# Kitware/SMQTK-Indexing

Measured on AMD Instinct MI355X. Metric: queries/sec, exact brute-force l2 kNN k=100 over 10000000x128 float32 (recall@100 = 1.0 by construction); scan HBM GB/s vs 8 TB/s peak, higher is better.
Workload: dtype f32 results (distances bit-identical to numpy float32); filter arithmetic int8 MFMA (i32 accumulation, measured per-row error bound), exact re-rank f32

## Files before the change

### smqtk_indexing_amd/csrc/sq_dense_i8.hpp

```cpp
#pragma once
#include "sq_dense_scan.hpp"

namespace sq {

typedef int i32x4 __attribute__((ext_vector_type(4)));
typedef int i32x16 __attribute__((ext_vector_type(16)));

template <int KS>
struct I8Geom {
    static constexpr int ROW_BYTES = KS * 32;
    static constexpr int UNIT_ROWS = KS == 4 ? 64 : 32;
    static constexpr int TILES = UNIT_ROWS / 32;
    static constexpr int UNIT_BYTES = UNIT_ROWS * ROW_BYTES;
    static constexpr int SLOT_BYTES = UNIT_BYTES + 256;
    static constexpr int WAVES = KS <= 8 ? 8 : 4;
    static constexpr int NSTAGE = 2;
    static constexpr int PIECES = UNIT_BYTES / 1024;
    static constexpr int SAMPLES_PER_UNIT = 2 * TILES;
};
static constexpr int I8_MAX_ROW_BYTES = 512;
__host__ __device__ constexpr int i8_row_bytes(int d) { return d <= 128 ? 128 : (d <= 256 ? 256 : 512); }
__host__ __device__ constexpr int i8_unit_rows(int row_bytes) { return row_bytes == 128 ? 64 : 32; }

__device__ __forceinline__ float i8_element(float v, const float* __restrict__ center, int k, bool cosine, double inv_norm) {
// ... 84 lines not shown
            }
        }
        if (__ballot(bad) != 0ull) continue;
#pragma unroll
        for (int c = 0; c < I8_NCLIP; ++c) {
            for (int o = 32; o > 0; o >>= 1) r2[c] += __shfl_xor(r2[c], o);
#pragma unroll
            for (int m = 0; m < I8_NCUT; ++m) cnt[c][m] += r2[c] > ca.cut[c][m] ? 1u : 0u;
        }
    }
    if (lane == 0) {
#pragma unroll
        for (int c = 0; c < I8_NCLIP; ++c)
#pragma unroll
            for (int m = 0; m < I8_NCUT; ++m)
                if (cnt[c][m]) atomicAdd(&counts[c * I8_NCUT + m], cnt[c][m]);
    }
}

template <int EPL>
static __global__ __launch_bounds__(256) void dense8_build_kernel(const float* __restrict__ db, long long n, long long ld, int d,
                                                                   long long n_pad, const float* __restrict__ center,
                                                                   const double* __restrict__ nx64, float inv_dx, float dx,
                                                                   signed char* __restrict__ out8, float* __restrict__ nrow,
                                                                   float* __restrict__ r2row, long long row_base, int row_bytes) {
    const int lane = threadIdx.x & 63;
    const long long row = row_base + (long long)blockIdx.x * 4 + (threadIdx.x >> 6);
    if (row >= n_pad) return;
    double e2 = 0.0, r2 = 0.0;
    bool finite = true;
    const double inv_norm = (row < n && nx64) ? 1.0 / sqrt(nx64[row]) : 1.0;
    for (int k0 = 0; k0 < row_bytes; k0 += 64 * EPL) {
        unsigned char q[EPL];
#pragma unroll
        for (int j = 0; j < EPL; ++j) q[j] = 0;
        if (row < n) {
#pragma unroll
            for (int j = 0; j < EPL; ++j) {
                const int k = k0 + EPL * lane + j;
                if (k < d) {
                    const float v = db[row * ld + k];
                    const float xc = i8_element(v, center, k, nx64 != nullptr, inv_norm);
                    if (!(xc == xc) || !(fabsf(xc) < 3.0e38f)) finite = false;
                    float t = rintf(xc * inv_dx);
                    t = fminf(fmaxf(t, -127.f), 127.f);
                    if (!(t == t)) t = 0.f;
                    q[j] = (unsigned char)(signed char)(int)t;
                    const double res = (double)xc - (double)t * (double)dx;
                    e2 += (double)xc * (double)xc;
                    r2 += res * res;
                }
            }
        }
        if (k0 + EPL * lane >= row_bytes) continue;
        unsigned char* dst = reinterpret_cast<unsigned char*>(out8) + row * row_bytes + k0 + EPL * lane;
        if constexpr (EPL == 2) {
            *reinterpret_cast<unsigned short*>(dst) = (unsigned short)(q[0] | (q[1] << 8));
        } else if constexpr (EPL == 4) {
            *reinterpret_cast<u32*>(dst) = (u32)q[0] | ((u32)q[1] << 8) | ((u32)q[2] << 16) | ((u32)q[3] << 24);
        } else {
            uint2 w;
            w.x = (u32)q[0] | ((u32)q[1] << 8) | ((u32)q[2] << 16) | ((u32)q[3] << 24);
            w.y = (u32)q[4] | ((u32)q[5] << 8) | ((u32)q[6] << 16) | ((u32)q[7] << 24);
            *reinterpret_cast<uint2*>(dst) = w;
        }
    }
    finite = __ballot(!finite) == 0ull;
    for (int o = 32; o > 0; o >>= 1) {
        e2 += __shfl_xor(e2, o);
        r2 += __shfl_xor(r2, o);
    }
    if (lane == 0) {
        float nr = __builtin_inff(), rr = 0.f;
        if (row < n && finite) {
            nr = nx64 ? 0.f : (float)e2;
            if ((double)nr > e2) nr = __uint_as_float(__float_as_uint(nr) - 1u);
            rr = (float)r2;
            if ((double)rr < r2) rr = __uint_as_float(__float_as_uint(rr) + 1u);
        }
        nrow[row] = nr;
        r2row[row] = rr;
    }
}

static __global__ __launch_bounds__(256) void dense8_resid_stats_kernel(const float* __restrict__ r2row, const float* __restrict__ nrow,
                                                                         long long n, double* __restrict__ sum_r2,
                                                                         u32* __restrict__ max_bits) {
    __shared__ double red[4];
    __shared__ float rmax[4], nmax[4];
    double acc = 0.0;
    float m = 0.f, mn = 0.f;
    for (long long i = (long long)blockIdx.x * 256 + threadIdx.x; i < n; i += (long long)gridDim.x * 256) {
        const float nv = nrow[i];
        if (nv < __builtin_inff() && nv > -__builtin_inff()) {
            const float v = r2row[i];
            acc += (double)v;
            m = fmaxf(m, v);
            mn = fmaxf(mn, nv);
        }
    }
    for (int o = 32; o > 0; o >>= 1) {
        acc += __shfl_xor(acc, o);
        m = fmaxf(m, __shfl_xor(m, o));
        mn = fmaxf(mn, __shfl_xor(mn, o));
    }
    if ((threadIdx.x & 63) == 0) {
        red[threadIdx.x >> 6] = acc;
        rmax[threadIdx.x >> 6] = m;
        nmax[threadIdx.x >> 6] = mn;
    }
    __syncthreads();
    if (threadIdx.x == 0) {
        atomicAdd(sum_r2, red[0] + red[1] + red[2] + red[3]);
        atomicMax(max_bits, __float_as_uint(fmaxf(fmaxf(rmax[0], rmax[1]), fmaxf(rmax[2], rmax[3]))));
        atomicMax(max_bits + 1, __float_as_uint(fmaxf(fmaxf(nmax[0], nmax[1]), fmaxf(nmax[2], nmax[3]))));
    }
}

static __global__ __launch_bounds__(256) void dense8_flag_kernel(const float* __restrict__ r2row, float* __restrict__ nrow, long long n,
                                                                  float r2_cut, u32* __restrict__ flagged, long long row_base) {
    const long long i = row_base + (long long)blockIdx.x * 256 + threadIdx.x;
    if (i >= n) return;
    if (nrow[i] < __builtin_inff() && r2row[i] > r2_cut) {
        nrow[i] = -__builtin_inff();
        atomicAdd(flagged, 1u);
    }
}

template <int EPL>
__device__ __forceinline__ void dense8_prep_query_row(const float* __restrict__ qrow, bool real, int d, const float* __restrict__ center,
                                                      double dx, double r_max, double x_max, int cosine,
                                                      signed char* __restrict__ p0, signed char* __restrict__ p1, float2& par_out,
                                                      double& qn2_out) {
    const int l16 = threadIdx.x & 15;
    const float sc = cosine ? -1.f : -2.f;
    float v[EPL][4];
#pragma unroll
    for (int c = 0; c < EPL; ++c)
#pragma unroll
        for (int e = 0; e < 4; ++e) {
            const int t = 64 * c + l16 + 16 * e;
            float raw = 0.f, cen = 0.f;
            if (real && t < d) {
                raw = qrow[t];
                if (center) cen = center[t];
            }
            v[c][e] = (real && t < d) ? (center ? __fsub_rn(raw, cen) : raw) : 0.f;
        }
    auto chunk_sum = [](double x0, double x1, double x2, double x3) __attribute__((always_inline)) {
        double sacc = (x0 + x2) + (x1 + x3);
        for (int o = 8; o > 0; o >>= 1) sacc += __shfl_xor(sacc, o);
        return sacc;
    };
    if (cosine) {
        double nn = 0.0;
#pragma unroll
        for (int c = 0; c < EPL; ++c)
            nn += chunk_sum((double)v[c][0] * (double)v[c][0], (double)v[c][1] * (double)v[c][1], (double)v[c][2] * (double)v[c][2],
                            (double)v[c][3] * (double)v[c][3]);
        const double rn = sqrt(nn);
#pragma unroll
        for (int c = 0; c < EPL; ++c)
#pragma unroll
            for (int e = 0; e < 4; ++e) v[c][e] = (float)((double)v[c][e] / rn);
    }
    double Q = 0.0;
    float mx = 0.f;
#pragma unroll
    for (int c = 0; c < EPL; ++c) {
        Q += chunk_sum((double)v[c][0] * (double)v[c][0], (double)v[c][1] * (double)v[c][1], (double)v[c][2] * (double)v[c][2],
                       (double)v[c][3] * (double)v[c][3]);
#pragma unroll
        for (int e = 0; e < 4; ++e) {
            float m = fabsf(sc * v[c][e]);
            if (!(m == m)) m = __builtin_inff();
            mx = fmaxf(mx, m);
        }
    }
    for (int o = 8; o > 0; o >>= 1) mx = fmaxf(mx, __shfl_xor(mx, o));
    const bool ok = real && mx < 3.0e38f && mx > 0.f;
    const double dq = ok ? (double)mx / 127.0 : 1.0;
    const double inv_dq = 1.0 / dq;
    double r2s = 0.0;
#pragma unroll
    for (int c = 0; c < EPL; ++c) {
        double r2[4];
#pragma unroll
        for (int e = 0; e < 4; ++e) {
            const double w = (double)(sc * v[c][e]);
            const double ws = w * inv_dq;
            float qt8 = 0.f, ql8 = 0.f;
            if (ok) {
                qt8 = fminf(fmaxf(rintf((float)ws), -127.f), 127.f);
                ql8 = fminf(fmaxf(rintf((float)((ws - (double)qt8) * 256.0)), -127.f), 127.f);
            }
            const int t = 64 * c + l16 + 16 * e;
            p0[t] = (signed char)(int)qt8;
            p1[t] = (signed char)(int)ql8;
            const double res = w - ((double)qt8 + (double)ql8 * 0.00390625) * dq;
            r2[e] = res * res;
        }
        r2s += chunk_sum(r2[0], r2[1], r2[2], r2[3]);
    }
    const double rq = sqrt(r2s) * (1.0 + 1e-9);
    const double unit = dx * dq;
    const double xr = x_max + r_max, qn = sqrt(Q), wn = (cosine ? 1.0 : 2.0) * qn;
    double e = r_max * wn + xr * rq + 4.0 * 5.9604644775390625e-08 * (xr * (wn + rq) + x_max * x_max);
    e *= 1.0 + 1e-6;
    float ef = (float)e;
    if ((double)ef < e) ef = __uint_as_float(__float_as_uint(ef) + 1u);
    if (!ok && real) ef = __builtin_inff();
    par_out = make_float2((float)unit, real ? ef : 0.f);
    qn2_out = real ? Q : 0.0;
}

template <int EPL>
static __global__ __launch_bounds__(64) void dense8_prep_queries_kernel(const float* __restrict__ q, int nq, int d,
                                                                         const float* __restrict__ center, double dx, double r_max,
                                                                         double x_max, signed char* __restrict__ qs8,
                                                                         float2* __restrict__ par, double* __restrict__ qn2,
                                                                         float* __restrict__ thr, u32* __restrict__ cnt,
                                                                         u32* __restrict__ oflag, float* __restrict__ q_al, int ldq,
                                                                         const DenseCallPtrs* __restrict__ ind, int cosine, int plane_rows) {
    constexpr int row_bytes = EPL * 64;
    if (ind) q = ind->q;
    const int qi = blockIdx.x * 4 + (threadIdx.x >> 4), t = threadIdx.x & 15;
    if (t == 0) {
        thr[qi] = qi < nq ? -__builtin_inff() : __builtin_nanf("");
        cnt[qi] = 0u;
        if (qi == 0) *oflag = 0u;
    }
    if (qi < nq)
        for (int i = t; i < ldq; i += 16) q_al[(long long)qi * ldq + i] = i < d ? q[(long long)qi * d + i] : 0.f;
    float2 pr;
    double Q;
    dense8_prep_query_row<EPL>(q + (long long)qi * d, qi < nq, d, center, dx, r_max, x_max, cosine,
                               qs8 + (long long)qi * row_bytes, qs8 + (long long)(plane_rows + qi) * row_bytes, pr, Q);
    if (t == 0) {
        par[qi] = pr;
        qn2[qi] = Q;
    }
}

struct Dense8ThrPost {
    const float2* par;
    const double* qn2;
    __device__ __forceinline__ void prologue(int, double*) const {}
    __device__ __forceinline__ float operator()(int q, float t) const {
        if (!(t < __builtin_inff())) return t;
        if (!(par[q].y < __builtin_inff())) return __builtin_nanf("");
        const double tt = (double)t + 2.0 * (double)par[q].y + 4e-6 * fabs((double)t + qn2[q]);
        float r = (float)tt;
        if ((double)r < tt) r = __uint_as_float(__float_as_uint(r) + (r >= 0.f ? 1 : -1));
        return r;
    }
};

struct Dense8ScanArgs {
    const signed char* scan8;
    const float* nrow;
    long long n;
    long long n_units;
    const signed char* qs8;
    const float2* par;
    const float* thr;
    uint2* wave_out;
    u32* wave_cnt;
    u32 wave_cap;
    float* sample_out;
    long long ns;
    long long unit_step;
    long long n_sel;
    int nrb;
    int nt;
    long long nt_from_row;
    int nqt;
    int plane_rows;
    int debug;
    float* wave_score;
    u32* hist;
};

template <int KS>
__device__ __forceinline__ int i8_swz(int c, int r) {
    if constexpr (KS == 4) return c ^ ((r >> 1) & 7);
    return (c & ~15) | ((c & 15) ^ (r & 15));
}

enum { I8_EMIT = 0, I8_SAMPLE = 1, I8_LANEMIN = 2, I8_EMIT_H = 3 };

static constexpr int I8_HIST_BINS = 64;
static constexpr int I8_CNT_SHIFT = 5;
static constexpr int I8_HIST_WORDS = TILE_ROWS * I8_HIST_BINS + (TILE_ROWS << I8_CNT_SHIFT);

template <int WAVES>
__device__ __forceinline__ void dense8_hist_flush(u32* lds_hist, u32* __restrict__ ghist) {
    constexpr int PER = TILE_ROWS * I8_HIST_BINS / WAVES;
    const int lane = threadIdx.x & 63;
    const int wave = __builtin_amdgcn_readfirstlane(threadIdx.x >> 6);
#pragma unroll
    for (int i = 0; i < PER / 64; ++i) {
        const int b = wave * PER + i * 64 + lane;
        const u32 v = __hip_atomic_exchange(lds_hist + b, 0u, __ATOMIC_RELAXED, __HIP_MEMORY_SCOPE_WORKGROUP);
        if (v) __hip_atomic_fetch_add(ghist + b, v, __ATOMIC_RELAXED, __HIP_MEMORY_SCOPE_AGENT);
    }
}

template <int KS, int MODE>
__device__ __forceinline__ void dense8_stream(const Dense8ScanArgs& a, unsigned char* smem, const i32x4 (&bq)[KS], const i32x4 (&bl)[KS],
                                              float unit_lo, float thr_l, u32& wcount, float& smin, u32* lds_ticket,
                                              float inv_w_l = 0.f, u32* lds_hist = nullptr) {
    using G = I8Geom<KS>;
    constexpr bool SAMPLE = MODE == I8_SAMPLE || MODE == I8_LANEMIN;
    const int lane = threadIdx.x & 63;
    const int wave = __builtin_amdgcn_readfirstlane(threadIdx.x >> 6);
    const int r31 = lane & 31, h = lane >> 5;
    const u32 lds_base = (u32)(uintptr_t)smem;
    const u32 ring_base = lds_base + (u32)wave * (G::NSTAGE * G::SLOT_BYTES);
    const unsigned char* ring_ptr = smem + wave * (G::NSTAGE * G::SLOT_BYTES);
    const long long wave_id = (long long)blockIdx.x * G::WAVES + wave;
    const long long nwaves = (long long)a.nrb * G::WAVES;
    uint2* wout = a.wave_out + wave_id * a.wave_cap;
    float* wsc = MODE == I8_EMIT_H ? a.wave_score + wave_id * a.wave_cap : nullptr;
    u32* hist_l = MODE == I8_EMIT_H ? lds_hist + r31 * I8_HIST_BINS : nullptr;

    const long long wg_first = (long long)blockIdx.x * G::WAVES;
    auto take_unit = [&]() __attribute__((always_inline)) -> long long {
        u32 t = 0;
        if (lane == 0) t = __hip_atomic_fetch_add(lds_ticket, 1u, __ATOMIC_RELAXED, __HIP_MEMORY_SCOPE_WORKGROUP);
        t = (u32)__builtin_amdgcn_readfirstlane((int)t);
        const long long u = wg_first + (long long)(t % G::WAVES) + (long long)(t / G::WAVES) * nwaves;
        return u < a.n_sel ? u : -1ll;
    };
    const long long my_units = wave_id < a.n_sel ? (a.n_sel - wave_id + nwaves - 1) / nwaves : 0;
    u32 voff[G::PIECES];
#pragma unroll
    for (int j = 0; j < G::PIECES; ++j) {
        const int lin = j * 1024 + lane * 16;
        const int r = lin / G::ROW_BYTES, cpos = (lin % G::ROW_BYTES) >> 4;
        voff[j] = (u32)(r * G::ROW_BYTES + i8_swz<KS>(cpos, r) * 16);
    }
    const u32 voff_n = (u32)lane * 4u;
    static_assert(G::NSTAGE == 2, "two ring slots: the units in flight are sel_even / sel_odd");
    long long issued = 0, sel_even = -1, sel_odd = -1;
    bool more = true;
    auto issue_next = [&]() __attribute__((always_inline)) {
        if (!more) return;
        const long long sel = take_unit();
        if (sel < 0) {
            more = false;
            return;
        }
        if (issued & 1) sel_odd = sel; else sel_even = sel;
        const long long unit_idx = sel * a.unit_step;
        const long long row0 = unit_idx * G::UNIT_ROWS;
        const u32 dst = ring_base + (u32)(issued % G::NSTAGE) * G::SLOT_BYTES;
        const unsigned char* base = reinterpret_cast<const unsigned char*>(a.scan8) + row0 * G::ROW_BYTES;
#pragma unroll
        for (int j = 0; j < G::PIECES; ++j) {
            if (a.nt && row0 >= a.nt_from_row)
                glds16<true>(base, voff[j], dst + (u32)j * 1024);
            else
                glds16<false>(base, voff[j], dst + (u32)j * 1024);
        }
        glds4(a.nrow + row0, voff_n, dst + G::UNIT_BYTES);
        ++issued;
    };
    for (int p = 0; p < G::NSTAGE; ++p) issue_next();
    const int flush_every = (int)(my_units >> 3) > 0 ? (int)(my_units >> 3) : 1;
    int to_flush = flush_every;

    for (long long it = 0; it < issued; ++it) {
        const long long sel = (it & 1) ? sel_odd : sel_even;
        const long long unit_idx = sel * a.unit_step;
        const long long row0 = unit_idx * G::UNIT_ROWS;
        wait_units_in_flight<G::NSTAGE, G::PIECES + 1>((int)(issued - it - 1));
        const unsigned char* sl = ring_ptr + (it % G::NSTAGE) * G::SLOT_BYTES;
        constexpr int KH = KS == 16 ? 8 : KS;
        i32x4 av[G::TILES][KH];
        f32x4 nr[G::TILES][4];
#pragma unroll
        for (int t = 0; t < G::TILES; ++t) {
            const int r = 32 * t + r31;
#pragma unroll
            for (int s = 0; s < KH; ++s)
                av[t][s] = *reinterpret_cast<const i32x4*>(sl + r * G::ROW_BYTES + i8_swz<KS>(2 * s + h, r) * 16);
#pragma unroll
            for (int c = 0; c < 4; ++c) nr[t][c] = *reinterpret_cast<const f32x4*>(sl + G::UNIT_BYTES + (32 * t + 8 * c + 4 * h) * 4);
        }
        asm volatile("s_waitcnt lgkmcnt(0)" ::: "memory");
        if constexpr (KS != 16) issue_next();
#pragma unroll
        for (int t = 0; t < G::TILES; ++t) {
            i32x16 acc, acl;
#pragma unroll
            for (int i = 0; i < 16; ++i) acc[i] = acl[i] = 0;
#pragma unroll
            for (int s = 0; s < KH; ++s) {
                acc = __builtin_amdgcn_mfma_i32_32x32x32_i8(av[t][s], bq[s], acc, 0, 0, 0);
                acl = __builtin_amdgcn_mfma_i32_32x32x32_i8(av[t][s], bl[s], acl, 0, 0, 0);
            }
            if constexpr (KS == 16) {
#pragma unroll
                for (int s = 0; s < KH; ++s)
                    av[t][s] = *reinterpret_cast<const i32x4*>(sl + r31 * G::ROW_BYTES + i8_swz<KS>(2 * (KH + s) + h, r31) * 16);
                asm volatile("s_waitcnt lgkmcnt(0)" ::: "memory");
                issue_next();
#pragma unroll
                for (int s = 0; s < KH; ++s) {
                    acc = __builtin_amdgcn_mfma_i32_32x32x32_i8(av[t][s], bq[KH + s], acc, 0, 0, 0);
                    acl = __builtin_amdgcn_mfma_i32_32x32x32_i8(av[t][s], bl[KH + s], acl, 0, 0, 0);
                }
            }
            if (a.debug & 1024) {
                if (acc[0] == 0x7fffffff && acl[5] == 0x7ffffffe) wcount += 1;
                continue;
            }
            float sc[16];
#pragma unroll
            for (int i = 0; i < 16; ++i) {
                float nv = nr[t][i >> 2][i & 3];
                if constexpr (SAMPLE) nv = nv == -__builtin_inff() ? __builtin_inff() : nv;
                sc[i] = __fmaf_rn((float)((acc[i] << 8) + acl[i]), unit_lo, nv);
            }
            float m = sc[0];
#pragma unroll
            for (int i = 1; i < 16; ++i) m = fminf(m, sc[i]);
            if constexpr (MODE == I8_LANEMIN) {
                smin = fminf(smin, m);
            } else if constexpr (MODE == I8_SAMPLE) {
                a.sample_out[(long long)r31 * a.ns + sel * G::SAMPLES_PER_UNIT + t * 2 + h] = m;
            } else {
                const u64 hit = __ballot(m <= thr_l);
                if (hit != 0) {
                    u32 mask = 0;
#pragma unroll
                    for (int i = 0; i < 16; ++i) mask |= (sc[i] <= thr_l ? 1u : 0u) << i;
                    const u64 bal = __ballot(mask != 0);
                    if (mask) {
                        const u32 pos = wcount + __builtin_amdgcn_mbcnt_hi((u32)(bal >> 32), __builtin_amdgcn_mbcnt_lo((u32)bal, 0u));
                        if (pos < a.wave_cap) {
                            wout[pos] = make_uint2((u32)(row0 + 32 * t + 4 * h), (mask << 16) | (u32)r31);
                            if constexpr (MODE == I8_EMIT_H) wsc[pos] = m;
                        }
                        if constexpr (MODE == I8_EMIT_H) {
                            if (m > -__builtin_inff()) {
                                const int bin = min((int)((thr_l - m) * inv_w_l), I8_HIST_BINS - 1);
                                __hip_atomic_fetch_add(hist_l + bin, 1u, __ATOMIC_RELAXED, __HIP_MEMORY_SCOPE_WORKGROUP);
                            }
                        }
                    }
                    wcount += (u32)__popcll(bal);
                }
            }
        }
        if constexpr (MODE == I8_EMIT_H) {
            if (--to_flush == 0) {
                to_flush = flush_every;
                dense8_hist_flush<G::WAVES>(lds_hist, a.hist);
            }
        }
    }
}

template <int KS>
__device__ __forceinline__ void dense8_load_planes(const signed char* planes, i32x4 (&bq)[KS], i32x4 (&bl)[KS]) {
    using G = I8Geom<KS>;
    const int lane = threadIdx.x & 63, r31 = lane & 31, h = lane >> 5;
#pragma unroll
    for (int s = 0; s < KS; ++s) {
        bq[s] = *reinterpret_cast<const i32x4*>(planes + r31 * G::ROW_BYTES + (2 * s + h) * 16);
        bl[s] = *reinterpret_cast<const i32x4*>(planes + (TILE_ROWS + r31) * G::ROW_BYTES + (2 * s + h) * 16);
    }
#pragma unroll
    for (int s = 0; s < KS; ++s) asm volatile("" : "+v"(bq[s]), "+v"(bl[s]));
}

template <int KS, bool SAMPLE>
__global__ __launch_bounds__(I8Geom<KS>::WAVES * 64, KS == 16 ? 1 : 2) void dense8_scan_kernel(Dense8ScanArgs a) {
    using G = I8Geom<KS>;
    extern __shared__ __attribute__((aligned(16))) unsigned char smem[];
    const int lane = threadIdx.x & 63;
    const int wave = __builtin_amdgcn_readfirstlane(threadIdx.x >> 6);
    const int r31 = lane & 31;
    i32x4 bq[KS], bl[KS];
    dense8_load_planes<KS>(a.qs8, bq, bl);
    float unit_lo = a.par[r31].x * 0.00390625f;
    float thr_l = SAMPLE ? 0.f : a.thr[r31];
    asm volatile("" : "+v"(unit_lo), "+v"(thr_l));
    u32 wcount = 0;
    float smin = 0.f;
    __shared__ u32 s_unit_ticket;
    if (threadIdx.x == 0) s_unit_ticket = 0u;
    __syncthreads();
    dense8_stream<KS, SAMPLE ? I8_SAMPLE : I8_EMIT>(a, smem, bq, bl, unit_lo, thr_l, wcount, smin, &s_unit_ticket);
    if constexpr (!SAMPLE) {
        if (lane == 0) {
            const long long wave_id = (long long)blockIdx.x * G::WAVES + wave;
            a.wave_cnt[2 * wave_id] = wcount;
            a.wave_cnt[2 * wave_id + 1] = 0u;
        }
    }
}


struct Dense8HeadArgs {
    Dense8ScanArgs s;
    const float* q;
    int nq, d;
    const float* center;
    double dx, r_max, x_max;
    int cosine;
    double* qn2;
    u32* cnt;
    u32* oflag;
    float* q_al;
    int ldq;
    const DenseCallPtrs* ind;
    float* lane_min;
    int keep;
    int kk;
};

template <int VM, int NQ>
__device__ __forceinline__ void wave_kth_smallest(const float* __restrict__ vals, long long stride, int M, int k, float (&out)[NQ]) {
    const int lane = threadIdx.x & 63;
    constexpr u32 KINF = 0xff800000u;
    u32 key[NQ][VM];
    u32 prefix[NQ];
    u32 xall = 0u;
#pragma unroll
    for (int n = 0; n < NQ; ++n) {
        u32 kmin = KINF, kmax = 0u;
#pragma unroll
        for (int j = 0; j < VM; ++j) {
            const int i = j * 64 + lane;
            u32 kv = ordered_f32(vals[n * stride + (i < M ? i : 0)]);
            kv = (i < M && kv < KINF) ? kv : KINF;
            key[n][j] = kv;
            kmin = kv < kmin ? kv : kmin;
            kmax = kv > kmax ? kv : kmax;
        }
        for (int o = 32; o > 0; o >>= 1) {
            const u32 a = (u32)__shfl_xor((int)kmin, o), b = (u32)__shfl_xor((int)kmax, o);
            kmin = a < kmin ? a : kmin;
            kmax = b > kmax ? b : kmax;
        }
        prefix[n] = __builtin_amdgcn_readfirstlane(kmin);
        xall |= __builtin_amdgcn_readfirstlane(kmin ^ kmax);
    }
    if (xall != 0u) {
        const int top = 31 - __clz((int)xall);
#pragma unroll
        for (int n = 0; n < NQ; ++n) prefix[n] &= ~((2u << top) - 1u);
        for (int b = top; b >= 0; --b) {
#pragma unroll
            for (int n = 0; n < NQ; ++n) {
                const u32 cand = prefix[n] | ((1u << b) - 1u);
                u32 c = 0;
#pragma unroll
                for (int j = 0; j < VM; ++j) c += (u32)__popcll(__ballot(key[n][j] <= cand));
                if (c < (u32)k) prefix[n] |= 1u << b;
            }
        }
    }
#pragma unroll
    for (int n = 0; n < NQ; ++n) {
        float r = unordered_f32(prefix[n]);
        if (prefix[n] >= KINF) {
            u32 c = 0;
#pragma unroll
            for (int j = 0; j < VM; ++j) c += (u32)__popcll(__ballot(key[n][j] < KINF));
            if (c < (u32)k) r = __builtin_inff();
        }
        out[n] = r;
    }
}

template <int KS>
__global__ __launch_bounds__(I8Geom<KS>::WAVES * 64, KS == 16 ? 1 : 2) void dense8_head_kernel(Dense8HeadArgs ha) {
    using G = I8Geom<KS>;
    constexpr int VB = G::WAVES * 2;
    extern __shared__ __attribute__((aligned(16))) unsigned char smem[];
    __shared__ float2 s_par[TILE_ROWS];
    __shared__ double s_qn2[TILE_ROWS];
    __shared__ float s_lm[TILE_ROWS][16];
    __shared__ u32 s_ticket, s_unit_ticket;
    if (threadIdx.x == 0) s_unit_ticket = 0u;
    const Dense8ScanArgs& a = ha.s;
    const int lane = threadIdx.x & 63;
    const int wave = __builtin_amdgcn_readfirstlane(threadIdx.x >> 6);
    const int r31 = lane & 31, h = lane >> 5;
    const float* q = ha.ind ? ha.ind->q : ha.q;
    const bool first = blockIdx.x == 0;
    signed char* planes = reinterpret_cast<signed char*>(smem);
#pragma unroll
    for (int rnd = 0; rnd < TILE_ROWS / (4 * G::WAVES); ++rnd) {
        const int qi = rnd * 4 * G::WAVES + wave * 4 + (lane >> 4);
        float2 pr;
        double Q;
        dense8_prep_query_row<KS / 2>(q + (long long)qi * ha.d, qi < ha.nq, ha.d, ha.center, ha.dx, ha.r_max, ha.x_max, ha.cosine,
                                      planes + qi * G::ROW_BYTES, planes + (TILE_ROWS + qi) * G::ROW_BYTES, pr, Q);
        if ((lane & 15) == 0) {
            s_par[qi] = pr;
            s_qn2[qi] = Q;
        }
        if (first) {
            if ((lane & 15) == 0) {
                const_cast<float2*>(a.par)[qi] = pr;
                ha.qn2[qi] = Q;
                ha.cnt[qi << I8_CNT_SHIFT] = 0u;
                if (qi == 0) ha.oflag[0] = 0u;
            }
            if (qi < ha.nq)
                for (int i = lane & 15; i < ha.ldq; i += 16) ha.q_al[(long long)qi * ha.ldq + i] = i < ha.d ? q[(long long)qi * ha.d + i] : 0.f;
        }
    }
    __syncthreads();
    i32x4 bq[KS], bl[KS];
    dense8_load_planes<KS>(planes, bq, bl);
    float unit_lo = s_par[r31].x * 0.00390625f;
    asm volatile("" : "+v"(unit_lo));
    if (first) {
        signed char* gp = const_cast<signed char*>(a.qs8);
        for (int i = threadIdx.x; i < 2 * TILE_ROWS * G::ROW_BYTES / 16; i += G::WAVES * 64)
            reinterpret_cast<uint4*>(gp)[i] = reinterpret_cast<const uint4*>(planes)[i];
        for (int i = threadIdx.x; i < I8_HIST_WORDS; i += G::WAVES * 64) a.hist[i] = 0u;
    }
    asm volatile("s_waitcnt vmcnt(0) lgkmcnt(0)" ::: "memory");
    __syncthreads();
    u32 wcount = 0;
    float smin = __builtin_inff();
    if (!(a.debug & 4096)) dense8_stream<KS, I8_LANEMIN>(a, smem, bq, bl, unit_lo, 0.f, wcount, smin, &s_unit_ticket);
    s_lm[r31][(wave * 2 + h) & 15] = smin;
    if (VB < 16 && wave == 0 && h == 0)
        for (int i = VB; i < 16; ++i) s_lm[r31][i] = __builtin_inff();
    __syncthreads();
    const int nb = (int)gridDim.x, keep = ha.keep, M = nb * keep;
#pragma unroll
    for (int rnd = 0; rnd < TILE_ROWS / (4 * G::WAVES); ++rnd) {
        const int qi = rnd * 4 * G::WAVES + wave * 4 + (lane >> 4), l16 = lane & 15;
        float v = s_lm[qi][l16];
#pragma unroll
        for (int kk2 = 2; kk2 <= 16; kk2 <<= 1)
#pragma unroll
            for (int j = kk2 >> 1; j > 0; j >>= 1) {
                const float o = __shfl_xor(v, j);
                const bool up = (l16 & kk2) == 0, lower = (l16 & j) == 0;
                v = (lower == up) ? fminf(v, o) : fmaxf(v, o);
            }
        if (l16 < keep) ha.lane_min[(long long)qi * M + (long long)blockIdx.x * keep + l16] = v;
    }
    asm volatile("s_waitcnt vmcnt(0)" ::: "memory");
    __syncthreads();
    if (threadIdx.x == 0) {
        __threadfence();
        const u32 t = atomicAdd(&ha.oflag[1], 1u);
        if (t == gridDim.x - 1) {
            __threadfence();
            ha.oflag[1] = 0u;
        }
        s_ticket = t;
    }
    __syncthreads();
    if (s_ticket != gridDim.x - 1) return;
    float* thr = const_cast<float*>(a.thr);
    const Dense8ThrPost post{s_par, s_qn2};
#pragma unroll
    for (int rnd = 0; rnd < TILE_ROWS / (4 * G::WAVES); ++rnd) {
        const int q0 = rnd * 4 * G::WAVES + wave * 4;
        float ts[4] = {-__builtin_inff(), -__builtin_inff(), -__builtin_inff(), -__builtin_inff()};
        if (q0 < ha.nq && !(a.debug & 2048)) {
            const float* v = ha.lane_min + (long long)q0 * M;
            if (M <= 256)
                wave_kth_smallest<4, 4>(v, M, M, ha.kk, ts);
            else if (M <= 512)
                wave_kth_smallest<8, 4>(v, M, M, ha.kk, ts);
            else if (M <= 1024)
                wave_kth_smallest<16, 4>(v, M, M, ha.kk, ts);
            else {
#pragma unroll
                for (int j = 0; j < 4; ++j) {
                    float one[1];
                    wave_kth_smallest<32, 1>(v + (long long)j * M, M, M, ha.kk, one);
                    ts[j] = one[0];
                }
            }
        }
#pragma unroll
        for (int j = 0; j < 4; ++j) {
            const float t = q0 + j < ha.nq ? post(q0 + j, ts[j]) : __builtin_nanf("");
            if (lane == 0) thr[q0 + j] = t;
        }
    }
}

struct Dense8TailArgs {
    const float* db;
    long long ld;
    int d;
    const float* q_al;
    int ldq, nq;
    void* keys;
    u32* cnt;
    u32 cap;
    u32* overflow;
    const double* nx64;
    const double* nq64;
    int debug;
    const double* qn2;
    int kk;
    int tighten;
    long long* clk;
};
static constexpr int I8_TAIL_QROWS_BYTES = 32 * (156 + 4) * 4;
static constexpr int I8_TAIL_LIST = 2048;
static constexpr int I8_TAIL_RERANK_BYTES = I8_TAIL_QROWS_BYTES + 3 * RERANK_MAX_GROUP * 4 + 8 * 32 * RERANK_STAGE_STRIDE * 4;
static constexpr int I8_TAIL_LDS_BYTES = I8_TAIL_RERANK_BYTES + I8_TAIL_LIST * 8 + TILE_ROWS * 4 + 16;

template <int KS, bool COSINE>
__global__ __launch_bounds__(I8Geom<KS>::WAVES * 64, KS == 16 ? 1 : 2) void dense8_body_kernel(Dense8ScanArgs a, Dense8TailArgs ta) {
    using G = I8Geom<KS>;
    static_assert(I8_TAIL_LDS_BYTES <= G::WAVES * G::NSTAGE * G::SLOT_BYTES, "the re-rank works in the ring's LDS");
    extern __shared__ __attribute__((aligned(16))) unsigned char smem[];
    __shared__ u32 s_hist8[TILE_ROWS * I8_HIST_BINS];
    __shared__ u32 s_wcnt[G::WAVES];
    __shared__ u32 s_unit_ticket;
    __shared__ float s_thr1[TILE_ROWS], s_eq[TILE_ROWS];
    __shared__ double s_qn2b[TILE_ROWS];
    __shared__ float2 s_parb[TILE_ROWS];
    if (threadIdx.x == 0) s_unit_ticket = 0u;
    if (threadIdx.x < TILE_ROWS) {
        s_thr1[threadIdx.x] = a.thr[threadIdx.x];
        s_parb[threadIdx.x] = a.par[threadIdx.x];
        s_eq[threadIdx.x] = a.par[threadIdx.x].y;
        s_qn2b[threadIdx.x] = ta.qn2[threadIdx.x];
    }
    const int lane = threadIdx.x & 63;
    const int wave = __builtin_amdgcn_readfirstlane(threadIdx.x >> 6);
    const int r31 = lane & 31;
    for (int i = threadIdx.x; i < TILE_ROWS * I8_HIST_BINS; i += G::WAVES * 64) s_hist8[i] = 0u;
    long long* clk = ta.clk ? ta.clk + (long long)blockIdx.x * 8 : nullptr;
    if (clk && threadIdx.x == 0) {
        clk[0] = (long long)wall_clock64();
        clk[1] = 0x7fffffffffffffffll;
    }
    __syncthreads();
    i32x4 bq[KS], bl[KS];
    dense8_load_planes<KS>(a.qs8, bq, bl);
    float unit_lo = a.par[r31].x * 0.00390625f;
    float thr_l = a.thr[r31];
    const float eq_l = a.par[r31].y;
    float inv_w_l = (eq_l > 0.f && eq_l < __builtin_inff()) ? 2.f / eq_l : 0.f;
    if (!(inv_w_l < 3.0e38f)) inv_w_l = 0.f;
    asm volatile("" : "+v"(unit_lo), "+v"(thr_l), "+v"(inv_w_l));
    u32 wcount = 0;
    float smin = 0.f;
    dense8_stream<KS, I8_EMIT_H>(a, smem, bq, bl, unit_lo, thr_l, wcount, smin, &s_unit_ticket, inv_w_l, s_hist8);
    const long long w0 = (long long)blockIdx.x * G::WAVES;
    if (lane == 0) {
        a.wave_cnt[2 * (w0 + wave)] = wcount;
        a.wave_cnt[2 * (w0 + wave) + 1] = 0u;
        s_wcnt[wave] = wcount;
        if (clk) atomicMin((unsigned long long*)(clk + 1), (unsigned long long)wall_clock64());
    }
    asm volatile("s_waitcnt vmcnt(0) lgkmcnt(0)" ::: "memory");
    __builtin_amdgcn_fence(__ATOMIC_RELEASE, "workgroup");
    __syncthreads();
    __builtin_amdgcn_fence(__ATOMIC_ACQUIRE, "workgroup");
    if (clk && threadIdx.x == 0) clk[2] = (long long)wall_clock64();
    float* fl = reinterpret_cast<float*>(smem);
    u32* su = reinterpret_cast<u32*>(smem + I8_TAIL_QROWS_BYTES);
    RerankLds L{fl, su, su + RERANK_MAX_GROUP, su + 2 * RERANK_MAX_GROUP,
                COSINE ? reinterpret_cast<float*>(smem + I8_TAIL_QROWS_BYTES + 3 * RERANK_MAX_GROUP * 4) : nullptr};
    {
        uint2* s_list = reinterpret_cast<uint2*>(smem + I8_TAIL_RERANK_BYTES);
        float* s_thr2 = reinterpret_cast<float*>(smem + I8_TAIL_RERANK_BYTES + I8_TAIL_LIST * 8);
        u32* s_npass = reinterpret_cast<u32*>(s_thr2 + TILE_ROWS);
        static_assert(I8_HIST_BINS == 64, "one lane per bin");
        bool any = false;
#pragma unroll
        for (int wi = 0; wi < G::WAVES; ++wi) any = any || s_wcnt[wi] != 0u;
        const Dense8ThrPost post{s_parb, s_qn2b};
        constexpr int NQW = TILE_ROWS / G::WAVES;
        u32 hc[NQW];
        if (ta.tighten && any) {
#pragma unroll
            for (int j = 0; j < NQW; ++j) {
                const int qi = (j >> 2) * 4 * G::WAVES + wave * 4 + (j & 3);
                hc[j] = __hip_atomic_load(a.hist + qi * I8_HIST_BINS + lane, __ATOMIC_RELAXED, __HIP_MEMORY_SCOPE_AGENT);
            }
#pragma unroll
            for (int j = 0; j < NQW; ++j) {
                const int qi = (j >> 2) * 4 * G::WAVES + wave * 4 + (j & 3);
                hc[j] += s_hist8[qi * I8_HIST_BINS + lane];
            }
        }
#pragma unroll
        for (int rnd = 0; rnd < TILE_ROWS / (4 * G::WAVES); ++rnd) {
#pragma unroll
            for (int j = 0; j < 4; ++j) {
                const int qi = rnd * 4 * G::WAVES + wave * 4 + j;
                const float t1 = s_thr1[qi];
                float t2 = t1;
                if (ta.tighten && any && qi < ta.nq && t1 < __builtin_inff() && t1 > -__builtin_inff()) {
                    u32 c = hc[rnd * 4 + j];
#pragma unroll
                    for (int o = 1; o < 64; o <<= 1) {
                        const u32 up = (u32)__shfl_down((int)c, o);
                        c += lane + o < 64 ? up : 0u;
                    }
                    const u64 reach = __ballot(c >= (u32)ta.kk);
                    const float eq = s_eq[qi];
                    if (reach != 0ull && eq > 0.f && eq < __builtin_inff()) {
                        const int jb = 63 - __clzll((long long)reach);
                        const float inv_w = 2.f / eq;
                        if (inv_w < 3.0e38f) {
                            const double t8 = (double)t1 - (double)jb / (double)inv_w * (1.0 - 1e-6);
                            float t8f = (float)t8;
                            if ((double)t8f < t8) t8f = __uint_as_float(__float_as_uint(t8f) + (t8f >= 0.f ? 1 : -1));
                            const float cand = post(qi, t8f);
                            if (cand < t2) t2 = cand;
                        }
                    }
                    if (lane == 0) atomicMax(a.hist + TILE_ROWS * I8_HIST_BINS + (qi << I8_CNT_SHIFT), ordered_f32(t2));
                }
                if (lane == 0) s_thr2[qi] = t2;
            }
        }
        if (ta.tighten) {
            L.scores = a.wave_score;
            L.thr2 = s_thr2;
            L.list = s_list;
            L.npass = s_npass;
            L.list_cap = I8_TAIL_LIST;
        }
        L.seg_cnt = s_wcnt;
        L.cnt_shift = I8_CNT_SHIFT;
        __syncthreads();
        if (clk && threadIdx.x == 0) clk[3] = (long long)wall_clock64();
        if (ta.tighten) dense8_hist_flush<G::WAVES>(s_hist8, a.hist);
    }
    using K = typename std::conditional<COSINE, K128, u64>::type;
    rerank_block<K, COSINE>(ta.db, ta.ld, ta.d, ta.q_al, ta.ldq, ta.nq, TILE_ROWS, a.wave_out, a.wave_cnt, a.wave_cap,
                            (long long)a.nrb * G::WAVES, G::WAVES, static_cast<K*>(ta.keys), ta.cnt, ta.cap, ta.overflow, ta.nx64,
                            ta.nq64, ta.debug, w0, L);
    if (clk) {
        asm volatile("s_waitcnt vmcnt(0) lgkmcnt(0)" ::: "memory");
        __syncthreads();
        if (threadIdx.x == 0) clk[4] = (long long)wall_clock64();
    }
}

template <int QT, bool SAMPLE>
__global__ __launch_bounds__(512, 2) void dense8_scan_mt_kernel(Dense8ScanArgs a) {
    using G = I8Geom<4>;
    extern __shared__ __attribute__((aligned(16))) unsigned char smem[];
    const int lane = threadIdx.x & 63;
    const int wave = __builtin_amdgcn_readfirstlane(threadIdx.x >> 6);
    const int r31 = lane & 31, h = lane >> 5;
    const u32 lds_base = (u32)(uintptr_t)smem;
    const u32 ring_base = lds_base + (u32)wave * (G::NSTAGE * G::SLOT_BYTES);
    const unsigned char* ring_ptr = smem + wave * (G::NSTAGE * G::SLOT_BYTES);
    const long long wave_id = (long long)blockIdx.x * G::WAVES + wave;
    uint2* wout = a.wave_out + wave_id * a.wave_cap;
    const int L = blockIdx.x;
    int grp, rb;
    if (a.nqt > 1) {
        const int xcd = L & 7, j = L >> 3;
        grp = j % a.nqt;
        rb = (j / a.nqt) * 8 + xcd;
    } else {
        grp = 0;
        rb = L;
    }
    const int q_first = grp * QT * TILE_ROWS;
    const long long rwave = (long long)rb * G::WAVES + wave, nwaves = (long long)a.nrb * G::WAVES;

    i32x4 bq[QT][4], bl[QT][4];
    float unit_lo[QT], thr_l[QT];
#pragma unroll
    for (int g = 0; g < QT; ++g) {
        const int qg = q_first + g * TILE_ROWS + r31;
#pragma unroll
        for (int s = 0; s < 4; ++s) {
            bq[g][s] = *reinterpret_cast<const i32x4*>(a.qs8 + (long long)qg * G::ROW_BYTES + (2 * s + h) * 16);
            bl[g][s] = *reinterpret_cast<const i32x4*>(a.qs8 + (long long)(a.plane_rows + qg) * G::ROW_BYTES + (2 * s + h) * 16);
        }
        unit_lo[g] = a.par[qg].x * 0.00390625f;
        thr_l[g] = SAMPLE ? 0.f : a.thr[qg];
        asm volatile("" : "+v"(unit_lo[g]), "+v"(thr_l[g]));
#pragma unroll
        for (int s = 0; s < 4; ++s) asm volatile("" : "+v"(bq[g][s]), "+v"(bl[g][s]));
    }

    const long long my_units = rwave < a.n_sel ? (a.n_sel - rwave + nwaves - 1) / nwaves : 0;
    u32 voff[G::PIECES];
#pragma unroll
    for (int j = 0; j < G::PIECES; ++j) {
        const int r = 8 * j + (lane >> 3);
        voff[j] = (u32)(r * G::ROW_BYTES + i8_swz<4>(lane & 7, r) * 16);
    }
    const u32 voff_n = (u32)lane * 4u;
    long long issued = 0;
    auto issue_next = [&]() __attribute__((always_inline)) {
        if (issued >= my_units) return;
        const long long unit_idx = (rwave + issued * nwaves) * a.unit_step;
        const long long row0 = unit_idx * G::UNIT_ROWS;
        const u32 dst = ring_base + (u32)(issued % G::NSTAGE) * G::SLOT_BYTES;
        const unsigned char* base = reinterpret_cast<const unsigned char*>(a.scan8) + row0 * G::ROW_BYTES;
#pragma unroll
        for (int j = 0; j < G::PIECES; ++j) {
            if (a.nt && row0 >= a.nt_from_row)
                glds16<true>(base, voff[j], dst + (u32)j * 1024);
            else
                glds16<false>(base, voff[j], dst + (u32)j * 1024);
        }
        glds4(a.nrow + row0, voff_n, dst + G::UNIT_BYTES);
        ++issued;
    };
    for (int p = 0; p < G::NSTAGE; ++p) issue_next();

    u32 wcount = 0;
    for (long long it = 0; it < my_units; ++it) {
        const long long unit_idx = (rwave + it * nwaves) * a.unit_step;
        const long long row0 = unit_idx * G::UNIT_ROWS;
        wait_units_in_flight<G::NSTAGE, G::PIECES + 1>((int)(issued - it - 1));
        const unsigned char* sl = ring_ptr + (it % G::NSTAGE) * G::SLOT_BYTES;
#pragma unroll
        for (int t = 0; t < 2; ++t) {
            const int r = 32 * t + r31;
            i32x4 av[4];
            f32x4 nr[4];
#pragma unroll
            for (int s = 0; s < 4; ++s) av[s] = *reinterpret_cast<const i32x4*>(sl + r * G::ROW_BYTES + i8_swz<4>(2 * s + h, r) * 16);
#pragma unroll
            for (int c = 0; c < 4; ++c) nr[c] = *reinterpret_cast<const f32x4*>(sl + G::UNIT_BYTES + (32 * t + 8 * c + 4 * h) * 4);
            asm volatile("s_waitcnt lgkmcnt(0)" ::: "memory");
            if (t == 1) issue_next();
#pragma unroll
            for (int g = 0; g < QT; ++g) {
                i32x16 acc, acl;
#pragma unroll
                for (int i = 0; i < 16; ++i) acc[i] = acl[i] = 0;
#pragma unroll
                for (int s = 0; s < 4; ++s) {
                    acc = __builtin_amdgcn_mfma_i32_32x32x32_i8(av[s], bq[g][s], acc, 0, 0, 0);
                    acl = __builtin_amdgcn_mfma_i32_32x32x32_i8(av[s], bl[g][s], acl, 0, 0, 0);
                }
                float sc[16];
#pragma unroll
                for (int i = 0; i < 16; ++i) {
                    float nv = nr[i >> 2][i & 3];
                    if constexpr (SAMPLE) nv = nv == -__builtin_inff() ? __builtin_inff() : nv;
                    sc[i] = __fmaf_rn((float)((acc[i] << 8) + acl[i]), unit_lo[g], nv);
                }
                float m = sc[0];
#pragma unroll
                for (int i = 1; i < 16; ++i) m = fminf(m, sc[i]);
                if constexpr (SAMPLE) {
                    const long long sel = rwave + it * nwaves;
                    a.sample_out[(long long)(q_first + g * TILE_ROWS + r31) * a.ns + sel * G::SAMPLES_PER_UNIT + t * 2 + h] = m;
                } else {
                    const u64 hit = __ballot(m <= thr_l[g]);
                    if (hit != 0) {
                        u32 mask = 0;
#pragma unroll
                        for (int i = 0; i < 16; ++i) mask |= (sc[i] <= thr_l[g] ? 1u : 0u) << i;
                        const u64 bal = __ballot(mask != 0);
                        if (mask) {
                            const u32 pos = wcount + __builtin_amdgcn_mbcnt_hi((u32)(bal >> 32), __builtin_amdgcn_mbcnt_lo((u32)bal, 0u));
                            if (pos < a.wave_cap) wout[pos] = make_uint2((u32)(row0 + 32 * t + 4 * h), (mask << 16) | (u32)(g * TILE_ROWS + r31));
                        }
                        wcount += (u32)__popcll(bal);
                    }
                }
            }
        }
    }
    if constexpr (!SAMPLE) {
        if (lane == 0) {
            a.wave_cnt[2 * wave_id] = wcount;
            a.wave_cnt[2 * wave_id + 1] = (u32)(grp * QT);
        }
    }
}

}
```

Before: 150,200.

## Software-pipeline int8 MFMA tiles with previous tile's epilogue for KS=4

For the 128-byte-row (KS=4) path, the loop now runs as a software pipeline. The MFMAs for the next tile are issued while the scalar epilogue of the previous tile runs (score computation, min reduction, ballot and candidate emission). Sched_group_barrier hints interleave one MFMA with eight VALU ops so the matrix and vector pipes overlap. The epilogue is factored into shared lambdas. The cost is extra live accumulator registers (two pairs of i32x16) and a more complex loop structure.

```diff
diff --git a/smqtk_indexing_amd/csrc/sq_dense_i8.hpp b/smqtk_indexing_amd/csrc/sq_dense_i8.hpp
--- a/smqtk_indexing_amd/csrc/sq_dense_i8.hpp
+++ b/smqtk_indexing_amd/csrc/sq_dense_i8.hpp
@@ -478,6 +478,126 @@
     const int flush_every = (int)(my_units >> 3) > 0 ? (int)(my_units >> 3) : 1;
     int to_flush = flush_every;
 
+    auto no_epilogue = [&](const i32x16& acc, const i32x16& acl) __attribute__((always_inline)) {
+        if (acc[0] == 0x7fffffff && acl[5] == 0x7ffffffe) wcount += 1;
+    };
+    auto epilogue = [&](const i32x16& acc, const i32x16& acl, const f32x4 (&nrt)[4], long long row_t, long long samp) __attribute__((always_inline)) {
+        float sc[16];
+#pragma unroll
+        for (int i = 0; i < 16; ++i) {
+            float nv = nrt[i >> 2][i & 3];
+            if constexpr (SAMPLE) nv = nv == -__builtin_inff() ? __builtin_inff() : nv;
+            sc[i] = __fmaf_rn((float)((acc[i] << 8) + acl[i]), unit_lo, nv);
+        }
+        float m = sc[0];
+#pragma unroll
+        for (int i = 1; i < 16; ++i) m = fminf(m, sc[i]);
+        if constexpr (MODE == I8_LANEMIN) {
+            smin = fminf(smin, m);
+        } else if constexpr (MODE == I8_SAMPLE) {
+            a.sample_out[(long long)r31 * a.ns + samp + h] = m;
+        } else {
+            const u64 hit = __ballot(m <= thr_l);
+            if (hit != 0) {
+                u32 mask = 0;
+#pragma unroll
+                for (int i = 15; i >= 0; --i) mask = mask + mask + (sc[i] <= thr_l ? 1u : 0u);
+                const u64 bal = __ballot(mask != 0);
+                if (mask) {
+                    const u32 pos = wcount + __builtin_amdgcn_mbcnt_hi((u32)(bal >> 32), __builtin_amdgcn_mbcnt_lo((u32)bal, 0u));
+                    if (pos < a.wave_cap) {
+                        wout[pos] = make_uint2((u32)(row_t + 4 * h), (mask << 16) | (u32)r31);
+                        if constexpr (MODE == I8_EMIT_H) wsc[pos] = m;
+                    }
+                    if constexpr (MODE == I8_EMIT_H) {
+                        if (m > -__builtin_inff()) {
+                            const int bin = min((int)((thr_l - m) * inv_w_l), I8_HIST_BINS - 1);
+                            __hip_atomic_fetch_add(hist_l + bin, 1u, __ATOMIC_RELAXED, __HIP_MEMORY_SCOPE_WORKGROUP);
+                        }
+                    }
+                }
+                wcount += (u32)__popcll(bal);
+            }
+        }
+    };
+    auto flush_tick = [&]() __attribute__((always_inline)) {
+        if constexpr (MODE == I8_EMIT_H) {
+            if (--to_flush == 0) {
+                to_flush = flush_every;
+                dense8_hist_flush<G::WAVES>(lds_hist, a.hist);
+            }
+        }
+    };
+
+    if constexpr (KS == 4) {
+        static_assert(G::TILES == 2, "the pipeline alternates a unit's two tiles");
+        i32x4 av[2][KS];
+        f32x4 nr[2][4];
+        auto load_unit = [&](long long it) __attribute__((always_inline)) {
+            wait_units_in_flight<G::NSTAGE, G::PIECES + 1>((int)(issued - it - 1));
+            const unsigned char* sl = ring_ptr + (it % G::NSTAGE) * G::SLOT_BYTES;
+#pragma unroll
+            for (int t = 0; t < 2; ++t) {
+                const int r = 32 * t + r31;
+#pragma unroll
+                for (int s = 0; s < KS; ++s)
+                    av[t][s] = *reinterpret_cast<const i32x4*>(sl + r * G::ROW_BYTES + i8_swz<KS>(2 * s + h, r) * 16);
+#pragma unroll
+                for (int c = 0; c < 4; ++c) nr[t][c] = *reinterpret_cast<const f32x4*>(sl + G::UNIT_BYTES + (32 * t + 8 * c + 4 * h) * 4);
+            }
+            asm volatile("s_waitcnt lgkmcnt(0)" ::: "memory");
+            issue_next();
+        };
+        auto mfma_tile = [&](const i32x4 (&avt)[KS], i32x16& acc, i32x16& acl) __attribute__((always_inline)) {
+#pragma unroll
+            for (int i = 0; i < 16; ++i) acc[i] = acl[i] = 0;
+#pragma unroll
+            for (int s = 0; s < KS; ++s) {
+                acc = __builtin_amdgcn_mfma_i32_32x32x32_i8(avt[s], bq[s], acc, 0, 0, 0);
+                acl = __builtin_amdgcn_mfma_i32_32x32x32_i8(avt[s], bl[s], acl, 0, 0, 0);
+            }
+        };
+        auto step = [&](const i32x4 (&avt)[KS], i32x16& acc_n, i32x16& acl_n, const i32x16& acc_p, const i32x16& acl_p,
+                        const f32x4 (&nrp)[4], long long row_p, long long samp_p) __attribute__((always_inline)) {
+            if (a.debug & 1024) {
+                mfma_tile(avt, acc_n, acl_n);
+                no_epilogue(acc_p, acl_p);
+                return;
+            }
+            mfma_tile(avt, acc_n, acl_n);
+            epilogue(acc_p, acl_p, nrp, row_p, samp_p);
+#pragma unroll
+            for (int i = 0; i < 2 * KS; ++i) {
+                __builtin_amdgcn_sched_group_barrier(0x008, 1, 0);
+                __builtin_amdgcn_sched_group_barrier(0x002, 8, 0);
+            }
+        };
+        if (issued > 0) {
+            i32x16 acc0, acl0, acc1, acl1;
+            f32x4 nr1[4];
+            long long row0 = sel_even * a.unit_step * G::UNIT_ROWS, samp = sel_even * G::SAMPLES_PER_UNIT;
+            load_unit(0);
+            mfma_tile(av[0], acc0, acl0);
+            for (long long it = 0;;) {
+                step(av[1], acc1, acl1, acc0, acl0, nr[0], row0, samp);
+#pragma unroll
+                for (int c = 0; c < 4; ++c) nr1[c] = nr[1][c];
+                const long long row1 = row0 + 32, samp1 = samp + 2;
+                flush_tick();
+                if (++it >= issued) {
+                    if (a.debug & 1024) no_epilogue(acc1, acl1); else epilogue(acc1, acl1, nr1, row1, samp1);
+                    break;
+                }
+                const long long sel = (it & 1) ? sel_odd : sel_even;
+                row0 = sel * a.unit_step * G::UNIT_ROWS;
+                samp = sel * G::SAMPLES_PER_UNIT;
+                load_unit(it);
+                step(av[0], acc0, acl0, acc1, acl1, nr1, row1, samp1);
+            }
+        }
+        return;
+    }
+
     for (long long it = 0; it < issued; ++it) {
         const long long sel = (it & 1) ? sel_odd : sel_even;
         const long long unit_idx = sel * a.unit_step;
@@ -521,53 +641,12 @@
                 }
             }
             if (a.debug & 1024) {
-                if (acc[0] == 0x7fffffff && acl[5] == 0x7ffffffe) wcount += 1;
+                no_epilogue(acc, acl);
                 continue;
             }
-            float sc[16];
-#pragma unroll
-            for (int i = 0; i < 16; ++i) {
-                float nv = nr[t][i >> 2][i & 3];
-                if constexpr (SAMPLE) nv = nv == -__builtin_inff() ? __builtin_inff() : nv;
-                sc[i] = __fmaf_rn((float)((acc[i] << 8) + acl[i]), unit_lo, nv);
-            }
-            float m = sc[0];
-#pragma unroll
-            for (int i = 1; i < 16; ++i) m = fminf(m, sc[i]);
-            if constexpr (MODE == I8_LANEMIN) {
-                smin = fminf(smin, m);
-            } else if constexpr (MODE == I8_SAMPLE) {
-                a.sample_out[(long long)r31 * a.ns + sel * G::SAMPLES_PER_UNIT + t * 2 + h] = m;
-            } else {
-                const u64 hit = __ballot(m <= thr_l);
-                if (hit != 0) {
-                    u32 mask = 0;
-#pragma unroll
-                    for (int i = 0; i < 16; ++i) mask |= (sc[i] <= thr_l ? 1u : 0u) << i;
-                    const u64 bal = __ballot(mask != 0);
-                    if (mask) {
-                        const u32 pos = wcount + __builtin_amdgcn_mbcnt_hi((u32)(bal >> 32), __builtin_amdgcn_mbcnt_lo((u32)bal, 0u));
-                        if (pos < a.wave_cap) {
-                            wout[pos] = make_uint2((u32)(row0 + 32 * t + 4 * h), (mask << 16) | (u32)r31);
-                            if constexpr (MODE == I8_EMIT_H) wsc[pos] = m;
-                        }
-                        if constexpr (MODE == I8_EMIT_H) {
-                            if (m > -__builtin_inff()) {
-                                const int bin = min((int)((thr_l - m) * inv_w_l), I8_HIST_BINS - 1);
-                                __hip_atomic_fetch_add(hist_l + bin, 1u, __ATOMIC_RELAXED, __HIP_MEMORY_SCOPE_WORKGROUP);
-                            }
-                        }
-                    }
-                    wcount += (u32)__popcll(bal);
-                }
-            }
-        }
-        if constexpr (MODE == I8_EMIT_H) {
-            if (--to_flush == 0) {
-                to_flush = flush_every;
-                dense8_hist_flush<G::WAVES>(lds_hist, a.hist);
-            }
-        }
+            epilogue(acc, acl, nr[t], row0 + 32 * t, sel * G::SAMPLES_PER_UNIT + t * 2);
+        }
+        flush_tick();
     }
 }
 
```

New measurement: 150,700 (median of 4 runs). No clear change (+0.4%).

## Prefetch unit tickets, use M0-based DMA issue, 32-bit indexing, swizzle histogram bins

Applied to the files above, without the earlier changes.

The stream loop now takes the next LDS ticket one iteration early and computes the next unit's base pointers ahead of time. Each async global-to-LDS copy sets M0 once per 8 pieces, with the slot offset folded into per-lane offsets and an immediate. Index arithmetic is narrowed from 64-bit to 32-bit. LDS histogram bins are XOR-swizzled by row to reduce atomic bank conflicts, with matching index changes in the flush and readback paths. This trims scalar and address overhead on the DMA issue path, but 32-bit row indices cap the supported row count and the swizzle must stay consistent everywhere the histogram is read.

```diff
diff --git a/smqtk_indexing_amd/csrc/sq_dense_i8.hpp b/smqtk_indexing_amd/csrc/sq_dense_i8.hpp
--- a/smqtk_indexing_amd/csrc/sq_dense_i8.hpp
+++ b/smqtk_indexing_amd/csrc/sq_dense_i8.hpp
@@ -410,7 +410,16 @@
     for (int i = 0; i < PER / 64; ++i) {
         const int b = wave * PER + i * 64 + lane;
         const u32 v = __hip_atomic_exchange(lds_hist + b, 0u, __ATOMIC_RELAXED, __HIP_MEMORY_SCOPE_WORKGROUP);
-        if (v) __hip_atomic_fetch_add(ghist + b, v, __ATOMIC_RELAXED, __HIP_MEMORY_SCOPE_AGENT);
+        if (v) __hip_atomic_fetch_add(ghist + (b ^ (b >> 6)), v, __ATOMIC_RELAXED, __HIP_MEMORY_SCOPE_AGENT);
+    }
+}
+
+template <int KS, bool NT, int J = 0>
+__device__ __forceinline__ void dense8_dma_unit(const void* base, const u32 (&voff_m)[I8Geom<KS>::PIECES], u32 dst) {
+    if constexpr (J < I8Geom<KS>::PIECES) {
+        if constexpr (J % 8 == 0) glds_set_m0(dst + (u32)(J * 1024 + 4096));
+        glds16_m0<(J % 8) * 1024 - 4096, NT>(base, voff_m[J]);
+        dense8_dma_unit<KS, NT, J + 1>(base, voff_m, dst);
     }
 }
 
@@ -426,63 +435,81 @@
     const u32 lds_base = (u32)(uintptr_t)smem;
     const u32 ring_base = lds_base + (u32)wave * (G::NSTAGE * G::SLOT_BYTES);
     const unsigned char* ring_ptr = smem + wave * (G::NSTAGE * G::SLOT_BYTES);
-    const long long wave_id = (long long)blockIdx.x * G::WAVES + wave;
-    const long long nwaves = (long long)a.nrb * G::WAVES;
-    uint2* wout = a.wave_out + wave_id * a.wave_cap;
-    float* wsc = MODE == I8_EMIT_H ? a.wave_score + wave_id * a.wave_cap : nullptr;
+    const u32 wave_id = blockIdx.x * G::WAVES + (u32)wave;
+    const u32 nwaves = (u32)a.nrb * G::WAVES;
+    const u32 n_sel = (u32)a.n_sel;
+    const u32 unit_step = SAMPLE ? (u32)a.unit_step : 1u;
+    uint2* wout = a.wave_out + (long long)wave_id * a.wave_cap;
+    float* wsc = MODE == I8_EMIT_H ? a.wave_score + (long long)wave_id * a.wave_cap : nullptr;
     u32* hist_l = MODE == I8_EMIT_H ? lds_hist + r31 * I8_HIST_BINS : nullptr;
 
-    const long long wg_first = (long long)blockIdx.x * G::WAVES;
-    auto take_unit = [&]() __attribute__((always_inline)) -> long long {
+    const u32 wg_first = blockIdx.x * G::WAVES;
+    u32 zero_v = 0;
+    asm volatile("" : "+v"(zero_v));
+    auto take_ticket = [&]() __attribute__((always_inline)) -> u32 {
         u32 t = 0;
-        if (lane == 0) t = __hip_atomic_fetch_add(lds_ticket, 1u, __ATOMIC_RELAXED, __HIP_MEMORY_SCOPE_WORKGROUP);
-        t = (u32)__builtin_amdgcn_readfirstlane((int)t);
-        const long long u = wg_first + (long long)(t % G::WAVES) + (long long)(t / G::WAVES) * nwaves;
-        return u < a.n_sel ? u : -1ll;
+        if (lane == 0) t = __hip_atomic_fetch_add(lds_ticket + zero_v, 1u, __ATOMIC_RELAXED, __HIP_MEMORY_SCOPE_WORKGROUP);
+        return t;
     };
-    const long long my_units = wave_id < a.n_sel ? (a.n_sel - wave_id + nwaves - 1) / nwaves : 0;
-    u32 voff[G::PIECES];
+    const u32 my_units = wave_id < n_sel ? (n_sel - wave_id + nwaves - 1) / nwaves : 0;
+    u32 voff_m[G::PIECES];
 #pragma unroll
     for (int j = 0; j < G::PIECES; ++j) {
         const int lin = j * 1024 + lane * 16;
         const int r = lin / G::ROW_BYTES, cpos = (lin % G::ROW_BYTES) >> 4;
-        voff[j] = (u32)(r * G::ROW_BYTES + i8_swz<KS>(cpos, r) * 16);
+        voff_m[j] = (u32)(r * G::ROW_BYTES + i8_swz<KS>(cpos, r) * 16) - (u32)((j % 8) * 1024 - 4096);
     }
     const u32 voff_n = (u32)lane * 4u;
-    static_assert(G::NSTAGE == 2, "two ring slots: the units in flight are sel_even / sel_odd");
-    long long issued = 0, sel_even = -1, sel_odd = -1;
+    static_assert(G::NSTAGE == 2, "two ring slots: the units in flight are sel_cur / sel_nxt");
+    int issued = 0;
+    u32 sel_cur = 0, sel_nxt = 0;
     bool more = true;
-    auto issue_next = [&]() __attribute__((always_inline)) {
+    u32 tick_v = take_ticket();
+    u32 n_sel_u = 0, n_row0 = 0;
+    const unsigned char* n_base = nullptr;
+    const float* n_nrow = nullptr;
+    bool n_nt = false;
+    auto prepare = [&]() __attribute__((always_inline)) {
         if (!more) return;
-        const long long sel = take_unit();
-        if (sel < 0) {
+        const u32 t = (u32)__builtin_amdgcn_readfirstlane((int)tick_v);
+        const u32 u = wg_first + t % G::WAVES + t / G::WAVES * nwaves;
+        if (u >= n_sel) {
             more = false;
             return;
         }
-        if (issued & 1) sel_odd = sel; else sel_even = sel;
-        const long long unit_idx = sel * a.unit_step;
-        const long long row0 = unit_idx * G::UNIT_ROWS;
-        const u32 dst = ring_base + (u32)(issued % G::NSTAGE) * G::SLOT_BYTES;
-        const unsigned char* base = reinterpret_cast<const unsigned char*>(a.scan8) + row0 * G::ROW_BYTES;
-#pragma unroll
-        for (int j = 0; j < G::PIECES; ++j) {
-            if (a.nt && row0 >= a.nt_from_row)
-                glds16<true>(base, voff[j], dst + (u32)j * 1024);
-            else
-                glds16<false>(base, voff[j], dst + (u32)j * 1024);
-        }
-        glds4(a.nrow + row0, voff_n, dst + G::UNIT_BYTES);
+        n_sel_u = u;
+        n_row0 = u * unit_step * G::UNIT_ROWS;
+        n_base = reinterpret_cast<const unsigned char*>(a.scan8) + (u64)n_row0 * G::ROW_BYTES;
+        n_nrow = a.nrow + n_row0;
+        n_nt = a.nt && (long long)n_row0 >= a.nt_from_row;
+    };
+    auto issue = [&]() __attribute__((always_inline)) {
+        if (!more) return;
+        const u32 dst = ring_base + (u32)(issued & 1) * G::SLOT_BYTES;
+        if (n_nt)
+            dense8_dma_unit<KS, true>(n_base, voff_m, dst);
+        else
+            dense8_dma_unit<KS, false>(n_base, voff_m, dst);
+        glds_set_m0(dst + G::UNIT_BYTES);
+        glds4_m0<0>(n_nrow, voff_n);
+        tick_v = take_ticket();
+        sel_nxt = n_sel_u;
         ++issued;
     };
-    for (int p = 0; p < G::NSTAGE; ++p) issue_next();
+    prepare();
+    issue();
+    sel_cur = sel_nxt;
+    prepare();
+    issue();
     const int flush_every = (int)(my_units >> 3) > 0 ? (int)(my_units >> 3) : 1;
     int to_flush = flush_every;
 
-    for (long long it = 0; it < issued; ++it) {
-        const long long sel = (it & 1) ? sel_odd : sel_even;
-        const long long unit_idx = sel * a.unit_step;
-        const long long row0 = unit_idx * G::UNIT_ROWS;
-        wait_units_in_flight<G::NSTAGE, G::PIECES + 1>((int)(issued - it - 1));
+    for (int it = 0; it < issued; ++it) {
+        const u32 sel = sel_cur;
+        sel_cur = sel_nxt;
+        const u32 row0 = sel * unit_step * G::UNIT_ROWS;
+        prepare();
+        wait_units_in_flight<G::NSTAGE, G::PIECES + 1>(issued - it - 1);
         const unsigned char* sl = ring_ptr + (it % G::NSTAGE) * G::SLOT_BYTES;
         constexpr int KH = KS == 16 ? 8 : KS;
         i32x4 av[G::TILES][KH];
@@ -497,7 +524,7 @@
             for (int c = 0; c < 4; ++c) nr[t][c] = *reinterpret_cast<const f32x4*>(sl + G::UNIT_BYTES + (32 * t + 8 * c + 4 * h) * 4);
         }
         asm volatile("s_waitcnt lgkmcnt(0)" ::: "memory");
-        if constexpr (KS != 16) issue_next();
+        if constexpr (KS != 16) issue();
 #pragma unroll
         for (int t = 0; t < G::TILES; ++t) {
             i32x16 acc, acl;
@@ -513,7 +540,7 @@
                 for (int s = 0; s < KH; ++s)
                     av[t][s] = *reinterpret_cast<const i32x4*>(sl + r31 * G::ROW_BYTES + i8_swz<KS>(2 * (KH + s) + h, r31) * 16);
                 asm volatile("s_waitcnt lgkmcnt(0)" ::: "memory");
-                issue_next();
+                issue();
 #pragma unroll
                 for (int s = 0; s < KH; ++s) {
                     acc = __builtin_amdgcn_mfma_i32_32x32x32_i8(av[t][s], bq[KH + s], acc, 0, 0, 0);
@@ -537,7 +564,7 @@
             if constexpr (MODE == I8_LANEMIN) {
                 smin = fminf(smin, m);
             } else if constexpr (MODE == I8_SAMPLE) {
-                a.sample_out[(long long)r31 * a.ns + sel * G::SAMPLES_PER_UNIT + t * 2 + h] = m;
+                a.sample_out[(long long)r31 * a.ns + (long long)sel * G::SAMPLES_PER_UNIT + t * 2 + h] = m;
             } else {
                 const u64 hit = __ballot(m <= thr_l);
                 if (hit != 0) {
@@ -548,13 +575,13 @@
                     if (mask) {
                         const u32 pos = wcount + __builtin_amdgcn_mbcnt_hi((u32)(bal >> 32), __builtin_amdgcn_mbcnt_lo((u32)bal, 0u));
                         if (pos < a.wave_cap) {
-                            wout[pos] = make_uint2((u32)(row0 + 32 * t + 4 * h), (mask << 16) | (u32)r31);
+                            wout[pos] = make_uint2(row0 + (u32)(32 * t + 4 * h), (mask << 16) | (u32)r31);
                             if constexpr (MODE == I8_EMIT_H) wsc[pos] = m;
                         }
                         if constexpr (MODE == I8_EMIT_H) {
                             if (m > -__builtin_inff()) {
                                 const int bin = min((int)((thr_l - m) * inv_w_l), I8_HIST_BINS - 1);
-                                __hip_atomic_fetch_add(hist_l + bin, 1u, __ATOMIC_RELAXED, __HIP_MEMORY_SCOPE_WORKGROUP);
+                                __hip_atomic_fetch_add(hist_l + (bin ^ r31), 1u, __ATOMIC_RELAXED, __HIP_MEMORY_SCOPE_WORKGROUP);
                             }
                         }
                     }
@@ -901,7 +928,7 @@
 #pragma unroll
             for (int j = 0; j < NQW; ++j) {
                 const int qi = (j >> 2) * 4 * G::WAVES + wave * 4 + (j & 3);
-                hc[j] += s_hist8[qi * I8_HIST_BINS + lane];
+                hc[j] += s_hist8[qi * I8_HIST_BINS + (lane ^ qi)];
             }
         }
 #pragma unroll
```

Result: no change. 148,600 before, 150,000 after, median of 6 (+0.9%).
